# zengyan-97/X2-VLM

Measured on AMD Instinct MI355X. Metric: image-text pairs/sec (fwd+bwd) X2VLM-base 224px bs=64/GPU, higher is better.
Workload: dtype bf16

## Files before the change

include/x2vlm_hip.h:

```cpp
#ifndef X2VLM_HIP_H
#define X2VLM_HIP_H
#include <stdint.h>
#ifdef __cplusplus
extern "C" {
#endif

const char* x2_last_error(void);
int x2_abi_version(void);
int x2_device_cus(void);
int x2_tune(int key, int value);
int x2_tune_get(int key);

int x2_gemm_nt(const void* A, const void* B, void* C, int M, int N, int K, int lda, int ldb, int ldc,
               const float* bias, const float* gamma, const float* resid, int ldr, void* aux, int ldaux,
               int act, int out_f32, unsigned drop_thr16, unsigned drop_seed, float drop_scale, const unsigned* drop_epoch,
               const float* rowscale, float* colsum, void* stream);

int x2_gemm_nt_dgelu_colparts(const void* A, const void* B, void* C, int M, int N, int K, int lda, int ldb, int ldc,
                              const void* aux, int ldaux, float* colparts, int* nrows_out, void* stream);
int x2_gemm_nt_splitk(const void* A, const void* B, float* C, int M, int N, int K, int lda, int ldb, int ldc,
                      int slices, float* ws, long ws_floats, void* stream);

int x2_gemm_tn_grouped(const int64_t* problems, int count, int accumulate, int split, float* ws, long ws_floats,
                       void* stream);
// ... 27 lines not shown

int x2_layernorm_fwd(const float* x, const float* w, const float* b, void* y_bf16, float* y_f32, float* mean,
                     float* rstd, int rows, int D, float eps, int period, unsigned drop_thr16, unsigned drop_seed,
                     float drop_scale, const unsigned* drop_epoch, void* stream);
int x2_layernorm_bwd(const void* dy , int dy_is_bf16, const float* x, const float* mean, const float* rstd, const float* w,
                     const float* dres, float* dx, void* dx_bf16, float* dw, float* db, float* dcol, int rows, int D,
                     int period, unsigned in_thr16, unsigned in_seed, float in_scale, unsigned out_thr16,
                     unsigned out_seed, float out_scale, const unsigned* drop_epoch, float* ws ,
                     int defer, int post, const float* post_rowscale, void* stream);
int x2_colsum_bf16(const void* y, float* out, int M, int N, int ld, float* ws , int defer, void* stream);
int x2_reduce_partials(const float* part, int nblk, int nk, int width, float* o0, float* o1, float* o2, void* stream);
int x2_reduce_partials_multi(const int64_t* desc, int count, void* stream);
int x2_layerscale_finish(const int64_t* desc, int count, void* stream);
int x2_rowscale_cast_colsum(const float* dx, const float* rowscale, void* dx_bf16, float* colsum, int M, int D,
                            float* ws , int defer, void* stream);
int x2_cast_bf16(const float* src, void* dst, long n, void* stream);
int x2_cast_transpose_bf16(const float* src, void* dst, void* dstT, int R, int C, int ldt, void* stream);
int x2_cast_transpose_multi(const int64_t* desc, int count, void* stream);
int x2_copy_f32_multi(const int64_t* desc, int count, void* stream);
int x2_patchify(const float* image, void* cols, int B, int R, int ps, void* stream);
int x2_assemble_tokens(const float* patch, const float* cls, float* x, int B, int P, int D, void* stream);
int x2_assemble_tokens_bwd(const float* dx, void* dpatch_bf16, float* dcls, int B, int P, int D, void* stream);
int x2_pool_tokens(float* x, const float* w, int B, int P, int D, int bwd, void* stream);
int x2_relpos_bias(const float* table, const long* index, const long* indexT , float* bias, float* biasT, int N, int H, int ld, int ldT,
                   float scale, void* stream);
int x2_relpos_bias_bwd(const void* dS, const int* inv_off, const int* inv_pos, float* dtable, int B, int N, int H, int ld,
                       int T, float* ws, int slices, void* stream);

int x2_embed_fwd(const long* ids, const float* word, const float* pos, const float* type0, float* out, int R, int L,
                 int D, void* stream);
int x2_embed_bwd(const long* ids, const float* g, float* dword, float* dpos, float* dtype0, int R, int L, int D,
                 float* scratch, void* stream);
int x2_gather_rows(const float* src, const int* idx, float* dst, void* dst_bf16, int R, long len, void* stream);
int x2_scatter_rows(const float* src, const int* idx, float* dst, int R, int D, long len, void* stream);
int x2_linear_f32(const float* A, const float* B, float* C, const float* bias, const float* alpha_ptr, float alpha,
                  int M, int N, int K, long sam, long sak, long sbn, long sbk, long ldc, int accumulate,
                  int ksplit ,
                  float* ws , void* stream);
int x2_l2norm(const float* x, const float* dy, float* out, int R, int D, int bwd, void* stream);
int x2_ce_fwd(const float* logits, long ld, const long* labels, int R, int C, float* lse, float* loss_row, float* out2,
              void* stream);
int x2_ce_bwd(const float* logits, long ld, const long* labels, const float* lse, const float* g, const float* stat,
              float gscale, int R, int C, float* dl_f32, void* dl_bf16, long ldd, void* stream);
int x2_mlm_ce_fwd(const void* X, const void* E, const float* bias, const long* labels, int R, int Vp, int V, int Hd,
                  int ldx, int lde, float* part, float* zlab, void* stream);
int x2_ce_combine(const float* part, int chunks, const float* zlab, const long* labels, int R, float* lse, float* loss_row,
                  float* out2, void* stream);
int x2_mlm_ce_bwd(const void* X, const void* E, const float* bias, const long* labels, const float* lse, const float* g,
                  const float* stat, float gscale, int R, int Vp, int V, int Hd, int ldx, int lde, void* dl_bf16, long ldd,
                  void* stream);
int x2_mask_tokens(const long* text_ids, const long* text_atts, int B, int L, const unsigned char* is_subword, int vocab,
                   const unsigned* words, int words_ld, unsigned seed, const unsigned* epoch, double mask_prob, int max_masks,
                   double skipgram_prb, int skipgram_size, int mask_whole_word, long cls_id, long mask_id, long pad_id, long pad_mask,
                   long* text_ids_masked, long* masked_pos, long* masked_ids, void* stream);
int x2_sample_negatives(const float* sim, int n, const long* group, const float* u, int* out, void* stream);
int x2_additive_mask(const long* atts, float* out, int S, int L, int Lp, float neg, void* stream);

// ... 40 lines not shown
```

probes/aten_count.py:

```python
import collections
import sqlite3
import sys

db = sqlite3.connect(sys.argv[1])
rows = list(db.execute("select name, start, end from kernels order by start"))
starts = [i for i, r in enumerate(rows) if r[0].startswith("patchify_kernel")]
a, b = starts[-2], starts[-1]
ours, aten = collections.Counter(), collections.Counter()
t_ours = t_aten = 0.0
for n, s, e in rows[a:b]:
    short = n.split("(")[0].replace("void ", "")
    if short.startswith("at::") or "rocclr" in short or short.startswith("Cijk") or "elementwise" in short:
        aten[short[:100]] += 1; t_aten += (e - s) / 1e3
    else:
        ours[short.split("<")[0]] += 1; t_ours += (e - s) / 1e3
print("# one step (the last complete one): %d launches, %d hand-written HIP (%.2f ms), %d ATen / runtime (%.3f ms)"
      % (b - a, sum(ours.values()), t_ours / 1e3, sum(aten.values()), t_aten / 1e3))
for n, k in aten.most_common():
    print("%4d  %s" % (k, n))
```

x2-vlm_amd/_lib.py:

```python
import ctypes as C
import os

import torch

_HERE = os.path.dirname(os.path.abspath(__file__))
LIB_PATH = os.environ.get("X2VLM_HIP_LIB") or os.path.join(_HERE, "libx2vlm_hip.so")

P, I, L, F, U = C.c_void_p, C.c_int, C.c_long, C.c_float, C.c_uint


class AttnArgs(C.Structure):
    _fields_ = [(n, P) for n in ("Q", "K", "V", "O", "dO", "Out", "dQ", "dK", "dV", "dS", "LSE", "Delta")] + \
               [(n, L) for n in ("q_bs", "q_rs", "k_bs", "k_rs", "v_bs", "v_rs", "o_bs", "o_rs",
                                 "dq_bs", "dq_rs", "dk_bs", "dk_rs", "dv_bs", "dv_rs", "do_bs", "do_rs")] + \
               [(n, I) for n in ("B", "Bkv", "H", "Lq", "Lk")] + [("scale", F)] + \
               [("bias", P), ("bias_ld", I), ("biasT", P), ("biasT_ld", I), ("mask", P), ("mask_ld", I),
                ("kv_idx", P), ("seq_off", P), ("seq_ids", P), ("ds_ld", I),
                ("drop_thr16", C.c_uint), ("drop_seed", C.c_uint), ("drop_scale", F), ("dbg", I), ("head_dim", I), ("drop_epoch", P),
                ("grid_nx", I), ("grid_ny", I), ("grid_nz", I), ("grid_map", I),
                ("phase", I), ("ws", P), ("ws_floats", L), ("colsum_ws", P)]


_SIGS = {
    "x2_gemm_nt": [P, P, P, I, I, I, I, I, I, P, P, P, I, P, I, I, I, U, U, F, P, P, P, P],
# ... 29 lines not shown
    "x2_ce_bwd": [P, L, P, P, P, P, F, I, I, P, P, L, P],
    "x2_mlm_ce_fwd": [P, P, P, P, I, I, I, I, I, I, P, P, P],
    "x2_ce_combine": [P, I, P, P, I, P, P, P, P],
    "x2_mlm_ce_bwd": [P, P, P, P, P, P, P, F, I, I, I, I, I, I, P, L, P],
    "x2_sample_negatives": [P, I, P, P, P, P],
    "x2_mask_tokens": [P, P, I, I, P, I, P, I, U, P, C.c_double, I, C.c_double, I, I, L, L, L, L, P, P, P, P],
    "x2_additive_mask": [P, P, I, I, I, F, P],
    "x2_kv_csr": [P, I, I, P, P, P],
    "x2_tail_index": [P, P, P, P, I, I, I, I, P, P, P, P, P],
    "x2_droppath_rows": [P, U, P, I, I, I, P, P],
    "x2_frame_mean": [P, P, P, P, P, I, I, I, I, I, P],
    "x2_gelu_f32": [P, P, P, L, P],
    "x2_grad_norm": [P, I, I, F, P, P, P],
    "x2_adamw_multi": [P, I, I, P, P, I, F, F, F, P, P],
    "x2_colsum_f32": [P, P, I, I, P],
    "x2_attn_fwd_mask2d": [C.POINTER(AttnArgs), P, I, P],
    "x2_attn_bwd_mask2d": [C.POINTER(AttnArgs), P, I, P],
    "x2_additive_mask2d": [P, P, I, I, I, F, P],
    "x2_embed_fwd_pid": [P, P, P, P, P, P, I, I, P],
    "x2_embed_bwd_pid": [P, P, P, P, P, P, I, I, I, P, P],
    "x2_mlm_ls_fwd": [P, P, P, P, L, I, I, I, I, I, I, P, P, P, P, P],
    "x2_ls_combine": [P, P, I, P, P, P, P, I, I, L, F, P, P, P, P],
    "x2_mlm_ls_bwd": [P, P, P, P, P, P, P, P, F, F, L, I, I, I, I, I, I, P, L, P],
}
_COMM_SIGS = {
    "x2_comm_unique_id": [P],
    "x2_comm_init": [P, I, I, C.POINTER(P)],
    "x2_comm_info": [P, C.POINTER(I), C.POINTER(I)],
    "x2_comm_allreduce_bucket": [P, P, L, I, I, P, P],
    "x2_comm_allgather": [P, P, P, L, I, P, P],
    "x2_comm_broadcast": [P, P, L, I, I, P, P],
    "x2_comm_destroy": [P],
}
EXPORTS = sorted(list(_SIGS) + list(_COMM_SIGS) + ["x2_last_error", "x2_abi_version", "x2_device_cus", "x2_tune", "x2_tune_get",
                                                         "x2_attn_bwd_one_pass"])

_lib = None


class X2HipError(RuntimeError):
    pass


def lib():
    global _lib
    if _lib is None:
# ... 42 lines not shown
```

x2-vlm_amd/csrc/heads.hip:

```cpp
#include "x2_common.h"
#define SCATTER_MAX_R_E 8192

__global__ __launch_bounds__(256) void embed_fwd_kernel(const long* __restrict__ ids, const float* __restrict__ word,
                                                        const float* __restrict__ pos, const float* __restrict__ type0,
                                                        float* __restrict__ out, int R, int L, int D) {
  const int r = blockIdx.x;
  const long id = ids[r];
  const int l = r % L;
  for (int d = threadIdx.x * 4; d < D; d += 1024) {
    const float4 a = *reinterpret_cast<const float4*>(word + id * D + d), b = *reinterpret_cast<const float4*>(pos + (long)l * D + d),
                 c = *reinterpret_cast<const float4*>(type0 + d);
    *reinterpret_cast<float4*>(out + (long)r * D + d) = float4{a.x + b.x + c.x, a.y + b.y + c.y, a.z + b.z + c.z, a.w + b.w + c.w};
  }
}
extern "C" int x2_embed_fwd(const long* ids, const float* word, const float* pos, const float* type0, float* out, int R, int L, int D,
                            void* stream) {
  X2_REQUIRE(R > 0 && L > 0 && D % 4 == 0, "x2_embed_fwd: R=%d L=%d D=%d", R, L, D);
  hipLaunchKernelGGL(embed_fwd_kernel, dim3(R), dim3(256), 0, (hipStream_t)stream, ids, word, pos, type0, out, R, L, D);
  return x2_check_launch("x2_embed_fwd");
}
__global__ __launch_bounds__(1024) void embed_bwd_word_kernel(const long* __restrict__ ids, const float* __restrict__ g, float* dword, int R,
                                                              int D) {
  __shared__ uint32_t bm[SCATTER_MAX_R_E / 32];
  __shared__ uint16_t lst[SCATTER_MAX_R_E];
// ... 79 lines not shown
  float* p = dpos + (long)l * D + d;
  p[0] += t.x; p[1] += t.y; p[2] += t.z; p[3] += t.w;
  *reinterpret_cast<float4*>(tot + (long)l * D + d) = t;
}
__global__ __launch_bounds__(64) void embed_bwd_type_kernel(const float* __restrict__ tot, float* dtype0, int L, int D) {
  const int d = (blockIdx.x * 64 + threadIdx.x) * 4;
  if (d >= D) return;
  float4 t{0.f, 0.f, 0.f, 0.f};
  for (int l = 0; l < L; ++l) { const float4 v = *reinterpret_cast<const float4*>(tot + (long)l * D + d); t.x += v.x; t.y += v.y; t.z += v.z; t.w += v.w; }
  float4 o = *reinterpret_cast<float4*>(dtype0 + d);
  o.x += t.x; o.y += t.y; o.z += t.z; o.w += t.w;
  *reinterpret_cast<float4*>(dtype0 + d) = o;
}
extern "C" int x2_embed_bwd(const long* ids, const float* g, float* dword, float* dpos, float* dtype0, int R, int L, int D, float* scratch,
                            void* stream) {
  X2_REQUIRE(R > 0 && L > 0 && D % 4 == 0 && D <= 4096 && scratch, "x2_embed_bwd: R=%d L=%d D=%d (D <= 4096, scratch of min(L, R) * D floats)", R, L, D);
  hipLaunchKernelGGL(embed_bwd_word_kernel, dim3(R), dim3(1024), 0, (hipStream_t)stream, ids, g, dword, R, D);
  const int Lp = L < R ? L : R;
  hipLaunchKernelGGL(embed_bwd_pos_kernel, dim3(Lp, (D / 4 + 255) / 256), dim3(256), 0, (hipStream_t)stream, g, dpos, scratch, R, L, D);
  hipLaunchKernelGGL(embed_bwd_type_kernel, dim3((D / 4 + 63) / 64), dim3(64), 0, (hipStream_t)stream, scratch, dtype0, Lp, D);
  return x2_check_launch("x2_embed_bwd");
}

__global__ __launch_bounds__(256) void gather_rows_kernel(const float* __restrict__ src, const int* __restrict__ idx, float* dst,
                                                          bf16_t* dstb, long len) {
  const long r = blockIdx.y;
  const float* s = src + (long)idx[r] * len;
  for (long e = (blockIdx.x * 256L + threadIdx.x) * 4; e < len; e += (long)gridDim.x * 1024) {
    const float4 v = *reinterpret_cast<const float4*>(s + e);
    if (dst) *reinterpret_cast<float4*>(dst + r * len + e) = v;
    if (dstb) *reinterpret_cast<u32x2*>(dstb + r * len + e) = u32x2{pack_bf16(v.x, v.y), pack_bf16(v.z, v.w)};
  }
}
extern "C" int x2_gather_rows(const float* src, const int* idx, float* dst, void* dst_bf16, int R, long len, void* stream) {
  X2_REQUIRE(R > 0 && len > 0 && len % 4 == 0, "x2_gather_rows: R=%d len=%ld", R, len);
  const int bx = (int)((len / 4 + 255) / 256 < 64 ? (len / 4 + 255) / 256 : 64);
  hipLaunchKernelGGL(gather_rows_kernel, dim3(bx, R), dim3(256), 0, (hipStream_t)stream, src, idx, dst, (bf16_t*)dst_bf16, len);
  return x2_check_launch("x2_gather_rows");
}
#define SCATTER_MAX_R 8192
__global__ __launch_bounds__(256) void scatter_rows_kernel(const float* __restrict__ src, const int* __restrict__ idx, float* __restrict__ dst,
                                                           int R, long len, int chunks) {
  __shared__ uint32_t bm[SCATTER_MAX_R / 32];
  const int d = blockIdx.x / chunks;
  const long e = ((long)(blockIdx.x % chunks) * 256L + threadIdx.x) * 4;
  float4 acc{0.f, 0.f, 0.f, 0.f};
// ... 501 lines not shown
```

x2-vlm_amd/csrc/rowwise.hip:

```cpp
#include "x2_common.h"

__device__ __forceinline__ long remap_row(int r, int period) { return period > 0 ? (long)r + r / period + 1 : r; }

#define LN_MAXV 8
#define LN_DISPATCH(D, CALL) do { const int nv_ = ((D) + 255) / 256; \
  if (nv_ <= 1) { CALL(1); } else if (nv_ == 2) { CALL(2); } else if (nv_ == 3) { CALL(3); } else if (nv_ == 4) { CALL(4); } \
  else if (nv_ <= 6) { CALL(6); } else { CALL(8); } } while (0)
template <int NV>
__global__ __launch_bounds__(256) void layernorm_fwd_kernel(const float* __restrict__ x, const float* __restrict__ w,
                                                            const float* __restrict__ bsh, bf16_t* yb, float* yf,
                                                            float* mean, float* rstd, int rows, int D, float eps, int period,
                                                            DropSpec drop_in_, const uint32_t* __restrict__ epoch) {
  const int row = blockIdx.x * 4 + (threadIdx.x >> 6), lane = threadIdx.x & 63;
  if (row >= rows) return;
  const DropSpec drop = drop_at_epoch(drop_in_, epoch);
  const long gr = remap_row(row, period);
  const float* xr = x + gr * D;
  float4 v[NV];
  float s = 0.f;
  const int nv = D >> 2;
#pragma unroll
  for (int i = 0; i < NV; ++i) {
    const int c = lane + i * 64;
    if (c < nv) { v[i] = *reinterpret_cast<const float4*>(xr + c * 4); s += v[i].x + v[i].y + v[i].z + v[i].w; }
// ... 648 lines not shown
}
__global__ __launch_bounds__(64) void cls_grad_kernel(const float* __restrict__ dx, float* dcls, int B, long bstride, int D) {
  const int d = (blockIdx.x * 64 + threadIdx.x) * 4;
  if (d >= D) return;
  float4 t{0.f, 0.f, 0.f, 0.f};
#pragma unroll 8
  for (int b = 0; b < B; ++b) {
    const float4 v = *reinterpret_cast<const float4*>(dx + b * bstride + d);
    t.x += v.x; t.y += v.y; t.z += v.z; t.w += v.w;
  }
  float4 o = *reinterpret_cast<float4*>(dcls + d);
  o.x += t.x; o.y += t.y; o.z += t.z; o.w += t.w;
  *reinterpret_cast<float4*>(dcls + d) = o;
}
extern "C" int x2_assemble_tokens_bwd(const float* dx, void* dpatch, float* dcls, int B, int P, int D, void* stream) {
  X2_REQUIRE(B > 0 && P > 0 && D % 4 == 0, "x2_assemble_tokens_bwd: B=%d P=%d D=%d", B, P, D);
  const long total = (long)B * (P + 1) * D / 4;
  const int blocks = (int)((total + 255) / 256 < 8192 ? (total + 255) / 256 : 8192);
  hipLaunchKernelGGL(assemble_tokens_bwd_kernel, dim3(blocks), dim3(256), 0, (hipStream_t)stream, dx, (bf16_t*)dpatch, dcls, B, P, D);
  hipLaunchKernelGGL(cls_grad_kernel, dim3((D / 4 + 63) / 64), dim3(64), 0, (hipStream_t)stream, dx, dcls, B, (long)(P + 1) * D, D);
  return x2_check_launch("x2_assemble_tokens_bwd");
}

__global__ __launch_bounds__(256) void pool_tokens_kernel(float* x, const float* __restrict__ w, int B, int P, int D, int bwd) {
  __shared__ float4 part[3][64];
  __shared__ float wpart[4];
  const int b = blockIdx.x, lane = threadIdx.x & 63, wave = threadIdx.x >> 6;
  const int d = (blockIdx.y * 64 + lane) * 4;
  const bool live = d < D;
  float* xb = x + (long)b * (P + 1) * D;
  float wsum = (float)P;
  if (w) {
    float s = 0.f;
    for (int p = threadIdx.x; p < P; p += 256) s += w[(long)b * P + p];
    s = wave_sum(s);
    if (lane == 0) wpart[wave] = s;
    __syncthreads();
    wsum = wpart[0] + wpart[1] + wpart[2] + wpart[3];
  }
  const float inv = 1.f / wsum;
  if (!bwd) {
    float4 acc{0.f, 0.f, 0.f, 0.f};
    if (live)
      for (int p = wave; p < P; p += 4) {
        const float wp = w ? w[(long)b * P + p] : 1.f;
        const float4 v = *reinterpret_cast<const float4*>(xb + (long)(1 + p) * D + d);
        acc.x += wp * v.x; acc.y += wp * v.y; acc.z += wp * v.z; acc.w += wp * v.w;
      }
    if (wave > 0) part[wave - 1][lane] = acc;
    __syncthreads();
    if (wave == 0 && live) {
#pragma unroll
      for (int k = 0; k < 3; ++k) { const float4 o = part[k][lane]; acc.x += o.x; acc.y += o.y; acc.z += o.z; acc.w += o.w; }
      *reinterpret_cast<float4*>(xb + d) = float4{acc.x * inv, acc.y * inv, acc.z * inv, acc.w * inv};
    }
  } else {
    if (live) {
      const float4 g0 = *reinterpret_cast<const float4*>(xb + d);
      for (int p = wave; p < P; p += 4) {
        const float wp = (w ? w[(long)b * P + p] : 1.f) * inv;
        float4 v = *reinterpret_cast<float4*>(xb + (long)(1 + p) * D + d);
        v.x += wp * g0.x; v.y += wp * g0.y; v.z += wp * g0.z; v.w += wp * g0.w;
        *reinterpret_cast<float4*>(xb + (long)(1 + p) * D + d) = v;
      }
    }
    __syncthreads();
    if (wave == 0 && live) *reinterpret_cast<float4*>(xb + d) = float4{0.f, 0.f, 0.f, 0.f};
  }
}
extern "C" int x2_pool_tokens(float* x, const float* w, int B, int P, int D, int bwd, void* stream) {
  X2_REQUIRE(B > 0 && P > 0 && D % 4 == 0, "x2_pool_tokens: B=%d P=%d D=%d", B, P, D);
  hipLaunchKernelGGL(pool_tokens_kernel, dim3(B, (D + 255) / 256), dim3(256), 0, (hipStream_t)stream, x, w, B, P, D, bwd);
  return x2_check_launch("x2_pool_tokens");
}

__global__ __launch_bounds__(256) void relpos_bias_kernel(const float* __restrict__ table, const long* __restrict__ index,
                                                          const long* __restrict__ indexT, float* bias, float* biasT, int N, int H,
                                                          int ld, int ldT, float scale) {
  const long total = (long)N * N;
  long e = blockIdx.x * 256L + threadIdx.x;
  if (e >= total) return;
  const int i = (int)(e / N), j = (int)(e % N);
  const long idx = index[e];
  if (indexT && biasT) {
    const long idt = indexT[e];
    for (int h = 0; h < H; ++h) {
      bias[((long)h * N + i) * ld + j] = table[idx * H + h] * scale;
      biasT[((long)h * N + i) * ldT + j] = table[idt * H + h] * scale;
    }
    return;
  }
  for (int h = 0; h < H; ++h) {
    const float v = table[idx * H + h] * scale;
    bias[((long)h * N + i) * ld + j] = v;
    if (biasT) biasT[((long)h * N + j) * ldT + i] = v;
  }
// ... 59 lines not shown
```

x2-vlm_amd/engine.py:

```python
import itertools
import math
import os
import weakref

import torch

from . import kernels as K
from ._lib import raw_stream

BF16, F32 = torch.bfloat16, torch.float32



_SERIAL = itertools.count(1)


def _tok(w):
    t = w.__dict__.get("_x2_serial")
    if t is None:
        t = w.__dict__["_x2_serial"] = next(_SERIAL)
    return t


class TScale:
# ... 434 lines not shown
            _count_call(("vit", id(p["blocks.%d.gamma_1" % i])))
        if stem:
            _count_call(("vit-stem", id(p["cls_token"])))
        ctx.meta, ctx.saved, ctx.final, ctx.cols = meta, saved, final, cols
        ctx.params = params
        ctx.dims = (B, P_, T, H, D, M, scale)
        return out

    @staticmethod
    def backward(ctx, dout):
        meta, params = ctx.meta, ctx.params
        BANK.note_backward()
        depth = meta["depth"]
        lo, hi = meta.get("lo", 0), meta.get("hi", depth)
        stem, head = lo == 0, hi == depth
        names = vision_param_names(depth, lo, hi)
        p = dict(zip(names, params))
        B, P_, T, H, D, M, scale = ctx.dims
        dev = dout.device
        out = {}
        if head:
            x_last, meanf, rstdf = ctx.final
            hn = ("fc_norm.weight", "fc_norm.bias")
            Gh = Grads(dev, [(n, p[n].shape, True) for n in hn], key=("vit-head", id(p["fc_norm.weight"])), params=[p[n] for n in hn])
            g = dout.contiguous().clone()
            K.pool_tokens(g, meta.get("pool_w"), bwd=True)
            dx, _ = K.layernorm_bwd(g.view(M, D), x_last, meanf, rstdf, p["fc_norm.weight"], Gh["fc_norm.weight"], Gh["fc_norm.bias"],
                                    period=P_)
            Gh.publish()
            out.update(Gh.g)
        else:
            dx = dout.contiguous().view(M, D)
        dS = torch.empty(B, H, T, K.round_up(T, 64), device=dev, dtype=BF16) if hi > lo else None
        F4 = p["blocks.%d.mlp.fc1.weight" % lo].shape[0] if hi > lo else 0
        dpath = meta.get("drop_path")
        pairs = _LayerPairs()
        arenas = {}
        for i in range(lo, hi):
            b = "blocks.%d." % i
            arenas[i] = Grads(dev, [("gamma_1", (D,), True), ("gamma_2", (D,), True), ("norm1.weight", (D,), True), ("norm1.bias", (D,), True),
                                    ("qkv_bias", (3 * D,), True), ("attn.relative_position_bias_table", p[b + "attn.relative_position_bias_table"].shape, True),
                                    ("attn.proj.bias", (D,), True), ("norm2.weight", (D,), True), ("norm2.bias", (D,), True),
                                    ("mlp.fc1.bias", (F4,), True), ("mlp.fc2.bias", (D,), True),
                                    ("_cs1", (D,), True), ("_cs2", (D,), True),
                                    ("attn.qkv.weight", (3 * D, D), False), ("attn.proj.weight", (D, D), False),
                                    ("mlp.fc1.weight", (F4, D), False), ("mlp.fc2.weight", (D, F4), False)], key=("vit", id(p[b + "gamma_1"])),
                              params=[p[n] for n in names if n.startswith(b)], zero=False)
        Gs = None
        if stem:
            sn = ("cls_token", "patch_embed.proj.weight", "patch_embed.proj.bias")
            Gs = Grads(dev, [(n, p[n].shape, True) for n in sn], key=("vit-stem", id(p["cls_token"])), params=[p[n] for n in sn], zero=False)
        Grads.zero_all(list(arenas.values()) + ([Gs] if Gs is not None else []))
        dxb = None
        for i in reversed(range(lo, hi)):
            b = "blocks.%d." % i
            rs1, rs2 = dpath[i] if dpath is not None else (None, None)
            (x, h1, mean1, rstd1, qkv, bias, biasT, att, lse, x1, h2, mean2, rstd2, pre, act) = ctx.saved[i - lo]
            ctx.saved[i - lo] = None
            G = arenas.pop(i)
            _begin_layer_backward()
            _, w2T = BANK.linear(p[b + "mlp.fc2.weight"], tscale=p[b + "gamma_2"])
            _, w1T = BANK.linear(p[b + "mlp.fc1.weight"])
            _, wprojT = BANK.linear(p[b + "attn.proj.weight"], tscale=p[b + "gamma_1"])
            _, wqkvT = BANK.linear(p[b + "attn.qkv.weight"])
            if dxb is None:
                dxb = K.rowscale_cast_colsum(dx, G["_cs2"], rowscale=rs2)
            if FUSE_DGELU_COLSUM:
                dpre = K.gemm_nt_dgelu_colsum(dxb, w2T, pre, G["mlp.fc1.bias"])
            else:
                dpre = K.gemm_nt(dxb, w2T, aux=pre, act=2)
                K.colsum_bf16(dpre, G["mlp.fc1.bias"])
            dh2 = K.gemm_nt(dpre, w1T)
            dx1, dx1b = K.layernorm_bwd(dh2, x1, mean2, rstd2, p[b + "norm2.weight"], G["norm2.weight"], G["norm2.bias"], dres=dx,
                                        post=(rs1, G["_cs1"]))
            datt = K.gemm_nt(dx1b, wprojT)
# ... 317 lines not shown



class EmbeddingsFn(torch.autograd.Function):

    @staticmethod
    def forward(ctx, ids, eps, drop, word, pos, typ, lnw, lnb, pids=None):
        S, L = ids.shape
        ids = ids.contiguous()
        if pids is not None:
            pids = pids.to(torch.int64).expand(S, L).contiguous()
            e = K.embed_fwd_pid(ids, pids, word.detach(), pos.detach(), typ.detach())
        else:
            e = K.embed_fwd(ids, word.detach(), pos.detach(), typ.detach())
        _, y, mean, rstd = K.layernorm_fwd(e, lnw, lnb, eps, want_bf16=False, want_f32=True, drop=drop)
        ctx.save_for_backward(ids, e, mean, rstd, word, pos, typ, lnw)
        ctx.drop, ctx.pids = drop, pids
        return y.view(S, L, -1)

    @staticmethod
    def backward(ctx, dy):
        ids, e, mean, rstd, word, pos, typ, lnw = ctx.saved_tensors
        n = lnw.numel()
        zeros = torch.zeros(2 * n + pos.numel() + typ.numel(), device=dy.device, dtype=F32)
        dw, db = zeros[:n], zeros[n:2 * n]
        dpos, dtyp = zeros[2 * n:2 * n + pos.numel()].view_as(pos), zeros[2 * n + pos.numel():].view_as(typ)
        de, _ = K.layernorm_bwd(dy.contiguous().view(e.shape), e, mean, rstd, lnw, dw, db, drop_in=ctx.drop)
        dword = _TIED_DWORD.pop(_tok(word), None)
        if dword is None:
            dword = torch.zeros_like(word)
        if ctx.pids is not None:
            K.embed_bwd_pid(ids, ctx.pids, de, dword, dpos, dtyp)
        else:
            K.embed_bwd(ids, de, dword, dpos, dtyp)
        return None, None, None, dword, dpos, dtyp, dw, db, None



class MlmLossFn(torch.autograd.Function):

    @staticmethod
    def forward(ctx, rows, labels, eps, keep_logits, dw_, db_, lnw, lnb, dec_bias, word, smooth=None):
        R, Hd = rows.shape
        V = word.shape[0]
        rb = K.cast_bf16(rows.contiguous())
        wd, _ = BANK.linear(dw_)
        t_pre = torch.empty(R, Hd, device=rows.device, dtype=BF16)
# ... 162 lines not shown
    @staticmethod
    def backward(ctx, g):
        logits, labels, lse, stat = ctx.saved_tensors
        return K.ce_bwd(logits, labels, lse, g.reshape(1).to(F32).contiguous(), stat), None


class GatherRowsFn(torch.autograd.Function):

    @staticmethod
    def forward(ctx, src, idx):
        src = src.contiguous()
        row_len = src[0].numel()
        ctx.save_for_backward(idx)
        ctx.shape = src.shape
        out, _ = K.gather_rows(src.view(src.shape[0], row_len), idx, row_len)
        return out.view((idx.numel(),) + src.shape[1:])

    @staticmethod
    def backward(ctx, dy):
        (idx,) = ctx.saved_tensors
        row_len = dy[0].numel()
        dst = K.scatter_rows(dy.contiguous().view(idx.numel(), row_len), idx, ctx.shape[0], row_len)
        return dst.view(ctx.shape), None
```

x2-vlm_amd/graph.py:

```python
import gc
import os

import torch

from . import kernels as K


class GraphedStep:
    def __init__(self, fn, warmup=2, enabled=True, verbose=False):
        self.fn, self.graph, self.out = fn, None, None
        self._grads = []
        self.stream = torch.cuda.Stream()
        self.mode = "eager"
        self.error = None
        self._epoch = None
        if not enabled or os.environ.get("X2_GRAPH", "1") == "0":
            return
        from . import engine
        if K.DROP_EPOCH is None:
            K.DROP_EPOCH = torch.zeros(1, dtype=torch.int32, device="cuda")
        self._epoch = K.DROP_EPOCH
        side_rule, engine.SIDE.only_from = engine.SIDE.only_from, self.stream.cuda_stream
        try:
            gc.collect()
# ... 271 lines not shown
        if hasattr(te, "cls"):
            eng.BANK.linear(te.cls.predictions.transform.dense.weight)
            eng.BANK.vocab(bert.embeddings.word_embeddings.weight)

    def _s_vision(self):
        b = self.batch
        enc = self.model.vision_encoder
        self.t["vmid"] = []
        enc.chunk_at, enc.chunk_hook = self.vcuts, self._vhook
        try:
            self.t["vis"] = self.model.tower_vision(b["image"], b.get("image_atts"), b.get("idx_to_group_img"), self.ret_bbox_loss)
        finally:
            enc.chunk_at, enc.chunk_hook = None, None

    def _s_feat(self):
        m = self.model
        if self.clamp_temp and isinstance(m.temp, torch.nn.Parameter):
            with torch.no_grad():
                m.temp.clamp_(0.001, 0.5)
        ie, _, full = self.t["vis"]
        self.t["ie"] = ie.detach().requires_grad_()
        self.t["full"] = None if full is None else full.detach().requires_grad_()
        self.t["both_leaf"] = self.t["both"].detach().requires_grad_()
        self.t["feat"] = m.tail_features(self.t["ie"], self.t["both_leaf"])

    def _gather(self):
        fi, ft = self.t["feat"]
        if not self.coll:
            for src, dst in ((fi, self.t["fi_all"]), (ft, self.t["ft_all"])):
                dst.detach().copy_(src.detach())
            return
        self.sG.wait_stream(self.sA)
        with torch.cuda.stream(self.sG):
            for src, dst in ((fi, self.t["fi_all"]), (ft, self.t["ft_all"])):
                out = dst.detach()
                if self.comm is not None:
                    self.comm.allgather(src.detach().contiguous(), out)
                else:
                    import torch.distributed as dist
                    dist.all_gather(list(out.chunk(self.world)), src.detach().contiguous(), group=self.pg)
                self.messages += 1
        self.sA.wait_stream(self.sG)

    def _s_loss(self):
        m, b, t = self.model, self.batch, self.t
        for leaf in (t["fi_all"], t["ft_all"], t["ie"], t["both_leaf"], t["full"]):
            if leaf is not None:
                leaf.grad = None
        fi, ft = t["feat"]
        loss = m.tail_losses(t["ie"], t["vis"][1], t["both_leaf"], fi, ft, b["text_atts"], b["masked_pos"], b["masked_ids"],
                             image_embeds_fullatts=t["full"], target_bbox=b.get("target_bbox"), is_image=b.get("is_image"),
                             ret_bbox_loss=self.ret_bbox_loss, ret_match_loss=self.ret_match_loss,
                             gathered=(t["fi_all"], t["ft_all"]))
        self._backward(loss)
        B = fi.shape[0]
        sl = slice(self.rank * B, (self.rank + 1) * B)
        if t["fi_all"].grad is not None:
            torch.autograd.backward([fi, ft], [t["fi_all"].grad[sl], t["ft_all"].grad[sl]])
        t["loss"] = {k: v.detach() for k, v in loss.items()}

    def _backward(self, losses):
        tot = self.total_loss(losses)
        if torch.is_tensor(tot) and tot.requires_grad:
            tot.backward()

    def _s_vision_bwd(self, ci=0):
        if ci == 0:
            ie_out, _, full_out = self.t["vis"]
            pairs = [(ie_out, self.t["ie"].grad)]
            if full_out is not None:
                pairs.append((full_out, self.t["full"].grad))
        else:
            x, leaf = self.t["vmid"][len(self.vcuts) - ci]
            pairs = [(x, leaf.grad)]
        pairs = [(o, g) for o, g in pairs if g is not None]
        if pairs:
            torch.autograd.backward([o for o, _ in pairs], [g for _, g in pairs])

    def _s_vision_wgrad(self, ci):
        work = self._vq.pop(ci, None)
        self._held.append(work)
# ... 399 lines not shown
```

x2-vlm_amd/kernels.py:

```python
import ctypes as C

import torch

from . import _lib
from ._lib import AttnArgs, call, ptr, raw_stream

BF16, F32 = torch.bfloat16, torch.float32


GEMM_TIMER = None


class _timed:

    def __init__(self, flops, name="gemm_nt"):
        self.flops = flops
        self.name = name

    def __enter__(self):
        if GEMM_TIMER is not None:
            self.a = torch.cuda.Event(enable_timing=True)
            self.b = torch.cuda.Event(enable_timing=True)
            self.a.record()

# ... 377 lines not shown


def assemble_tokens(patch, cls, B, P):
    D = patch.shape[1]
    x = torch.empty(B, P + 1, D, device=patch.device, dtype=F32)
    call("x2_assemble_tokens", ptr(patch), ptr(cls), ptr(x), B, P, D)
    return x


def assemble_tokens_bwd(dx, dcls):
    B, T, D = dx.shape
    dpatch = torch.empty(B * (T - 1), D, device=dx.device, dtype=BF16)
    call("x2_assemble_tokens_bwd", ptr(dx), ptr(dpatch), ptr(dcls), B, T - 1, D)
    return dpatch


def pool_tokens(x, w=None, bwd=False):
    B, T, D = x.shape
    assert x.dtype == F32 and x.is_contiguous() and (w is None or (w.dtype == F32 and w.shape == (B, T - 1) and w.is_contiguous()))
    call("x2_pool_tokens", ptr(x), ptr(w), B, T - 1, D, 1 if bwd else 0)
    return x


LOG2E = 1.4426950408889634


def relpos_bias(table, index, want_T=True, log2=False):
    N = index.shape[0]
    H = table.shape[1]
    ld = round_up(N, 64)
    bias = torch.empty(H, N, ld, device=table.device, dtype=F32)
    biasT = torch.empty(H, N, ld, device=table.device, dtype=F32) if want_T else None
    call("x2_relpos_bias", ptr(table), ptr(index), ptr(_relpos_index_t(index)) if want_T else None, ptr(bias), ptr(biasT), N, H, ld, ld,
         LOG2E if log2 else 1.0)
    return bias, biasT


_RELPOS_CSR = {}
_RELPOS_T = {}


def _relpos_index_t(index):
    key = (index.data_ptr(), index._version)
    ent = _RELPOS_T.get(key)
    if ent is None:
        ent = _RELPOS_T[key] = (index.t().contiguous(), index)
# ... 301 lines not shown
```

x2-vlm_amd/model_pretrain.py:

```python
import torch

from . import kernels as K
from . import ops
from .xvlm import XVLMBase


class XVLM(XVLMBase):
    def __init__(self, config, load_vision_params=True, load_text_params=True, pretraining=True):
        super().__init__(config, load_vision_params=load_vision_params, load_text_params=load_text_params,
                         use_contrastive_loss=True, use_matching_loss=True, use_mlm_loss=True, use_bbox_loss=True,
                         config_text=None, pretraining=pretraining)
        self.overlap_towers = True
        self._text_stream = None

    def tower_text(self, text_ids, text_atts, text_ids_masked):
        return self.get_text_embeds(torch.cat([text_ids, text_ids_masked]), torch.cat([text_atts, text_atts]))

    def tower_vision(self, image, image_atts=None, idx_to_group_img=None, ret_bbox_loss=False):
        if ret_bbox_loss:
            return self.get_vision_embeds(image, image_atts=image_atts, idx_to_group_img=idx_to_group_img)
        return self.get_vision_embeds(image) + (None,)

    def tail_features(self, image_embeds, both):
        return self.get_features(image_embeds, both[:image_embeds.shape[0]])

    def tail_losses(self, image_embeds, image_atts, both, image_feat, text_feat, text_atts, masked_pos, masked_ids,
                    image_embeds_fullatts=None, target_bbox=None, is_image=None, ret_bbox_loss=False, ret_match_loss=True,
                    gathered=None):
        B = image_embeds.shape[0]
        dev = both.device
        text_embeds = both[:B]
        loss_itc = self.get_contrastive_loss(image_feat, text_feat, gathered=gathered)
        ineg, tneg = self.get_hard_negatives(image_feat, text_feat) if ret_match_loss else (None, None)
        if both.is_cuda:
            t_idx, kv, atts, enc_atts = K.tail_index(ineg, tneg, text_atts.contiguous(), image_atts.contiguous(), with_match=ret_match_loss)
        else:
            ar = torch.arange(B, device=dev, dtype=torch.int32)
            t_idx, kv = (torch.cat([ar, ar, tneg, ar + B]), torch.cat([ar, ineg, ar, ar])) if ret_match_loss else (ar + B, ar)
            atts, enc_atts = torch.cat([text_atts, text_atts])[t_idx.long()], image_atts[kv.long()]
        h0 = ops.gather_rows(both, t_idx)
        fused = self.get_cross_embeds(image_embeds, enc_atts, text_embeds=h0, text_atts=atts, kv_idx=kv)
        if ret_match_loss:
            loss_itm = self._itm_loss(fused[:3 * B, 0, :], B)
        else:
            loss_itm = torch.tensor(0.0)
        loss_mlm, self.last_mlm_lse, self.last_mlm_logits = self.text_encoder.mlm_loss_from_hidden(fused[-B:], masked_pos, masked_ids)
        loss = {"loss_itc": loss_itc, "loss_itm": loss_itm, "loss_mlm": loss_mlm}
        self.last = dict(image_embeds=image_embeds.detach(), text_embeds=text_embeds.detach(), image_feat=image_feat.detach(),
                         text_feat=text_feat.detach())
        if ret_bbox_loss:
            output_coord = self.predict_bbox(image_embeds_fullatts, text_embeds, text_atts)
            self.last["bbox_coord"] = output_coord.detach()
            loss["loss_bbox"], loss["loss_giou"] = self.get_bbox_loss(output_coord, target_bbox, is_image=is_image)
        return loss

    def forward_multimodal(self, image, text_ids, text_atts, text_ids_masked=None, masked_pos=None, masked_ids=None,
                           image_atts=None, idx_to_group_img=None, target_bbox=None, is_image=None,
                           ret_bbox_loss=False, ret_match_loss=True):
        overlap = self.overlap_towers and image.is_cuda
        if overlap:
            if self._text_stream is None:
                self._text_stream = torch.cuda.Stream()
            main = torch.cuda.current_stream()
            self._text_stream.wait_stream(main)
            with torch.cuda.stream(self._text_stream):
                both = self.tower_text(text_ids, text_atts, text_ids_masked)
        image_embeds, image_atts, image_embeds_fullatts = self.tower_vision(image, image_atts, idx_to_group_img, ret_bbox_loss)
        if overlap:
            main.wait_stream(self._text_stream)
# ... 22 lines not shown
```

Baseline: 2970.

## Replace ATen slicing/clone/zero ops around heads with custom fused HIP kernels

Adds custom kernels to remove leftover ATen launches: pool-token backward now writes to a separate buffer and zeroes the dx row in the same pass, which replaces the clone. Slicing the fused output into CLS rows and the MLM tail now goes through a custom autograd function, so backward is one kernel instead of ATen scatter and zero-fill. The ITC features take CLS leaves, with a token-0 add into the tower grads. Embedding grad zeroing now goes through the batched zero_all, and probes are added to list the ATen call sites. This cuts the number of small launches per step, at the cost of more custom paths that must keep gradients exact.

```diff
diff --git a/include/x2vlm_hip.h b/include/x2vlm_hip.h
--- a/include/x2vlm_hip.h
+++ b/include/x2vlm_hip.h
@@ -73,6 +73,7 @@
 int x2_assemble_tokens(const float* patch, const float* cls, float* x, int B, int P, int D, void* stream);
 int x2_assemble_tokens_bwd(const float* dx, void* dpatch_bf16, float* dcls, int B, int P, int D, void* stream);
 int x2_pool_tokens(float* x, const float* w, int B, int P, int D, int bwd, void* stream);
+int x2_pool_tokens_bwd_to(const float* g, float* out, float* zero0, const float* w, int B, int P, int D, void* stream);
 int x2_relpos_bias(const float* table, const long* index, const long* indexT , float* bias, float* biasT, int N, int H, int ld, int ldT,
                    float scale, void* stream);
 int x2_relpos_bias_bwd(const void* dS, const int* inv_off, const int* inv_pos, float* dtable, int B, int N, int H, int ld,
@@ -84,6 +85,8 @@
                  float* scratch, void* stream);
 int x2_gather_rows(const float* src, const int* idx, float* dst, void* dst_bf16, int R, long len, void* stream);
 int x2_scatter_rows(const float* src, const int* idx, float* dst, int R, int D, long len, void* stream);
+int x2_split_tokens_bwd(const float* dcls, const float* dtail, float* out, int S, int n_cls, int L, int D, void* stream);
+int x2_add_token0(float* x, const float* rows, int B, int T, int D, void* stream);
 int x2_linear_f32(const float* A, const float* B, float* C, const float* bias, const float* alpha_ptr, float alpha,
                   int M, int N, int K, long sam, long sak, long sbn, long sbk, long ldc, int accumulate,
                   int ksplit ,
diff --git a/probes/aten_count.py b/probes/aten_count.py
--- a/probes/aten_count.py
+++ b/probes/aten_count.py
@@ -3,18 +3,25 @@
 import sys
 
 db = sqlite3.connect(sys.argv[1])
-rows = list(db.execute("select name, start, end from kernels order by start"))
+rows = list(db.execute("select name, start, end, stream_id from kernels order by start"))
 starts = [i for i, r in enumerate(rows) if r[0].startswith("patchify_kernel")]
 a, b = starts[-2], starts[-1]
 ours, aten = collections.Counter(), collections.Counter()
 t_ours = t_aten = 0.0
-for n, s, e in rows[a:b]:
+listing, prev = [], "-"
+for n, s, e, sid in rows[a:b]:
     short = n.split("(")[0].replace("void ", "")
     if short.startswith("at::") or "rocclr" in short or short.startswith("Cijk") or "elementwise" in short:
         aten[short[:100]] += 1; t_aten += (e - s) / 1e3
+        listing.append("%8.3f ms %6.1f us  stream %s  %-72s after %s" % ((s - rows[a][1]) / 1e6, (e - s) / 1e3, sid,
+                                                                          short.replace("at::native::", "")[:72], prev))
     else:
         ours[short.split("<")[0]] += 1; t_ours += (e - s) / 1e3
+        prev = short.split("<")[0]
 print("# one step (the last complete one): %d launches, %d hand-written HIP (%.2f ms), %d ATen / runtime (%.3f ms)"
       % (b - a, sum(ours.values()), t_ours / 1e3, sum(aten.values()), t_aten / 1e3))
 for n, k in aten.most_common():
     print("%4d  %s" % (k, n))
+if "--list" in sys.argv[2:]:
+    print("# offset, duration, stream, kernel, preceding hand-written kernel")
+    print("\n".join(listing))
diff --git a/probes/aten_sites.py b/probes/aten_sites.py
--- /dev/null
+++ b/probes/aten_sites.py
@@ -0,0 +1,82 @@
+import argparse
+import collections
+import importlib
+import os
+import sys
+import tempfile
+import traceback
+
+import torch
+from torch.utils._python_dispatch import TorchDispatchMode
+
+ROOT = os.path.dirname(os.path.dirname(os.path.abspath(__file__)))
+sys.path.insert(0, ROOT)
+import bench
+
+NO_KERNEL = ("empty", "new_empty", "empty_like", "empty_strided", "detach", "alias", "record_stream", "_local_scalar_dense", "lift_fresh",
+             "is_pinned", "_to_copy.host")
+
+
+def main():
+    ap = argparse.ArgumentParser()
+    ap.add_argument("--config", default="base")
+    args = ap.parse_args()
+    conf = bench.CONFIGS[args.config]
+    dev = torch.device("cuda", 0)
+    mp = importlib.import_module("x2-vlm_amd.model_pretrain")
+    cfgs = importlib.import_module("x2-vlm_amd.configs")
+    graph = importlib.import_module("x2-vlm_amd.graph")
+    synth = importlib.import_module("x2-vlm_amd.synthetic")
+    torch.manual_seed(0)
+    cfg = cfgs.pretrain_config(tempfile.mkdtemp(), conf["size"], conf["res"])
+    model = mp.XVLM(config=cfg, load_vision_params=False, load_text_params=False, pretraining=True).to(dev)
+    model.train()
+    batch = {k: v.to(dev) for k, v in bench.synthetic_batch(0, conf["batch"], 30, conf["res"], frames=conf["frames"]).items()}
+    masking = synth.masking_config({}, synth.synth_subword_flags(30522).to(dev), seed=1234)
+    runner = graph.SegmentedStep(model, batch, warmup=2, enabled=False, masking=masking)
+
+    seg = ["-"]
+    inner = runner._seg
+
+    def _seg(mode, name, stream, fn, pool):
+        seg[0] = name
+        try:
+            inner(mode, name, stream, fn, pool)
+        finally:
+            seg[0] = "between"
+    runner._seg = _seg
+    rec = collections.OrderedDict()
+
+    class Rec(TorchDispatchMode):
+        def __torch_dispatch__(self, func, types, args=(), kwargs=None):
+            out = func(*args, **(kwargs or {}))
+            name = str(func).replace("aten.", "")
+            if any(r.alias_info is not None and not r.alias_info.is_write for r in func._schema.returns) or name.split(".")[0] in NO_KERNEL:
+                return out
+            outs = out if isinstance(out, (tuple, list)) else (out,)
+            ts = [t for t in outs if torch.is_tensor(t)]
+            if not any(t.is_cuda for t in ts) and not any(torch.is_tensor(a) and a.is_cuda for a in args):
+                return out
+            site = "(autograd engine)"
+            for fr in reversed(traceback.extract_stack()):
+                if "x2-vlm_amd" in fr.filename:
+                    site = "%s:%d" % (os.path.basename(fr.filename), fr.lineno)
+                    break
+            nbytes = sum(t.numel() * t.element_size() for t in ts)
+            key = (seg[0], name, site, nbytes, " ".join("x".join(map(str, t.shape)) or "scalar" for t in ts))
+            rec[key] = rec.get(key, 0) + 1
+            return out
+
+    with Rec():
+        runner()
+    torch.cuda.synchronize()
+    print("# segment | op | site | output bytes | output shape | calls")
+    tot = collections.Counter()
+    for (s, name, site, nbytes, shape), n in rec.items():
+        print("%-8s %-28s %-24s %10d  %-18s x%d" % (s, name, site, nbytes, shape, n))
+        tot[s] += n
+    print("# ops per segment: " + ", ".join("%s %d" % kv for kv in tot.items()))
+
+
+if __name__ == "__main__":
+    main()
diff --git a/x2-vlm_amd/_lib.py b/x2-vlm_amd/_lib.py
--- a/x2-vlm_amd/_lib.py
+++ b/x2-vlm_amd/_lib.py
@@ -75,6 +75,9 @@
     "x2_mlm_ls_fwd": [P, P, P, P, L, I, I, I, I, I, I, P, P, P, P, P],
     "x2_ls_combine": [P, P, I, P, P, P, P, I, I, L, F, P, P, P, P],
     "x2_mlm_ls_bwd": [P, P, P, P, P, P, P, P, F, F, L, I, I, I, I, I, I, P, L, P],
+    "x2_pool_tokens_bwd_to": [P, P, P, P, I, I, I, P],
+    "x2_split_tokens_bwd": [P, P, P, I, I, I, I, P],
+    "x2_add_token0": [P, P, I, I, I, P],
 }
 _COMM_SIGS = {
     "x2_comm_unique_id": [P],
diff --git a/x2-vlm_amd/csrc/heads.hip b/x2-vlm_amd/csrc/heads.hip
--- a/x2-vlm_amd/csrc/heads.hip
+++ b/x2-vlm_amd/csrc/heads.hip
@@ -125,6 +125,45 @@
   return x2_check_launch("x2_embed_bwd");
 }
 
+__global__ __launch_bounds__(256) void split_tokens_bwd_kernel(const float* __restrict__ dcls, const float* __restrict__ dtail, float* __restrict__ out,
+                                                               int S, int n_cls, int L, int D) {
+  const long total = (long)S * L * D / 4;
+  const long st = (long)gridDim.x * 256;
+  for (long i = blockIdx.x * 256L + threadIdx.x; i < total; i += st) {
+    const long e = i * 4;
+    const int d = (int)(e % D);
+    const long row = e / D;
+    const int l = (int)(row % L), s = (int)(row / L);
+    float4 v{0.f, 0.f, 0.f, 0.f};
+    if (s >= n_cls) { if (dtail) v = *reinterpret_cast<const float4*>(dtail + e - (long)n_cls * L * D); }
+    else if (l == 0 && dcls) v = *reinterpret_cast<const float4*>(dcls + (long)s * D + d);
+    *reinterpret_cast<float4*>(out + e) = float4{v.x + 0.f, v.y + 0.f, v.z + 0.f, v.w + 0.f};
+  }
+}
+extern "C" int x2_split_tokens_bwd(const float* dcls, const float* dtail, float* out, int S, int n_cls, int L, int D, void* stream) {
+  X2_REQUIRE(out && S > 0 && L > 0 && D > 0 && D % 4 == 0 && n_cls >= 0 && n_cls <= S, "x2_split_tokens_bwd: S=%d n_cls=%d L=%d D=%d", S, n_cls, L, D);
+  const long total = (long)S * L * D / 4;
+  const int blocks = (int)((total + 255) / 256 < 8192 ? (total + 255) / 256 : 8192);
+  hipLaunchKernelGGL(split_tokens_bwd_kernel, dim3(blocks), dim3(256), 0, (hipStream_t)stream, dcls, dtail, out, S, n_cls, L, D);
+  return x2_check_launch("x2_split_tokens_bwd");
+}
+
+__global__ __launch_bounds__(256) void add_token0_kernel(float* x, const float* __restrict__ rows, int B, long bstride, int D) {
+  const long i = (blockIdx.x * 256L + threadIdx.x) * 4;
+  if (i >= (long)B * D) return;
+  const int b = (int)(i / D), d = (int)(i % D);
+  float4 a = *reinterpret_cast<float4*>(x + b * bstride + d);
+  const float4 r = *reinterpret_cast<const float4*>(rows + i);
+  a.x += r.x; a.y += r.y; a.z += r.z; a.w += r.w;
+  *reinterpret_cast<float4*>(x + b * bstride + d) = a;
+}
+extern "C" int x2_add_token0(float* x, const float* rows, int B, int T, int D, void* stream) {
+  X2_REQUIRE(x && rows && B > 0 && T > 0 && D > 0 && D % 4 == 0, "x2_add_token0: x=%p rows=%p B=%d T=%d D=%d", (void*)x, (const void*)rows, B, T, D);
+  const long n4 = (long)B * D / 4;
+  hipLaunchKernelGGL(add_token0_kernel, dim3((unsigned)((n4 + 255) / 256)), dim3(256), 0, (hipStream_t)stream, x, rows, B, (long)T * D, D);
+  return x2_check_launch("x2_add_token0");
+}
+
 __global__ __launch_bounds__(256) void gather_rows_kernel(const float* __restrict__ src, const int* __restrict__ idx, float* dst,
                                                           bf16_t* dstb, long len) {
   const long r = blockIdx.y;
diff --git a/x2-vlm_amd/csrc/rowwise.hip b/x2-vlm_amd/csrc/rowwise.hip
--- a/x2-vlm_amd/csrc/rowwise.hip
+++ b/x2-vlm_amd/csrc/rowwise.hip
@@ -694,13 +694,15 @@
   return x2_check_launch("x2_assemble_tokens_bwd");
 }
 
-__global__ __launch_bounds__(256) void pool_tokens_kernel(float* x, const float* __restrict__ w, int B, int P, int D, int bwd) {
+__global__ __launch_bounds__(256) void pool_tokens_kernel(const float* src, float* x, float* zero0, const float* __restrict__ w, int B, int P,
+                                                          int D, int bwd) {
   __shared__ float4 part[3][64];
   __shared__ float wpart[4];
   const int b = blockIdx.x, lane = threadIdx.x & 63, wave = threadIdx.x >> 6;
   const int d = (blockIdx.y * 64 + lane) * 4;
   const bool live = d < D;
   float* xb = x + (long)b * (P + 1) * D;
+  const float* sb = src + (long)b * (P + 1) * D;
   float wsum = (float)P;
   if (w) {
     float s = 0.f;
@@ -728,22 +730,30 @@
     }
   } else {
     if (live) {
-      const float4 g0 = *reinterpret_cast<const float4*>(xb + d);
+      const float4 g0 = *reinterpret_cast<const float4*>(sb + d);
       for (int p = wave; p < P; p += 4) {
         const float wp = (w ? w[(long)b * P + p] : 1.f) * inv;
-        float4 v = *reinterpret_cast<float4*>(xb + (long)(1 + p) * D + d);
+        float4 v = *reinterpret_cast<const float4*>(sb + (long)(1 + p) * D + d);
         v.x += wp * g0.x; v.y += wp * g0.y; v.z += wp * g0.z; v.w += wp * g0.w;
         *reinterpret_cast<float4*>(xb + (long)(1 + p) * D + d) = v;
       }
     }
     __syncthreads();
-    if (wave == 0 && live) *reinterpret_cast<float4*>(xb + d) = float4{0.f, 0.f, 0.f, 0.f};
+    if (wave == 0 && live) {
+      *reinterpret_cast<float4*>(xb + d) = float4{0.f, 0.f, 0.f, 0.f};
+      if (zero0) *reinterpret_cast<float4*>(zero0 + (long)b * (P + 1) * D + d) = float4{0.f, 0.f, 0.f, 0.f};
+    }
   }
 }
 extern "C" int x2_pool_tokens(float* x, const float* w, int B, int P, int D, int bwd, void* stream) {
-  X2_REQUIRE(B > 0 && P > 0 && D % 4 == 0, "x2_pool_tokens: B=%d P=%d D=%d", B, P, D);
-  hipLaunchKernelGGL(pool_tokens_kernel, dim3(B, (D + 255) / 256), dim3(256), 0, (hipStream_t)stream, x, w, B, P, D, bwd);
+  X2_REQUIRE(x && B > 0 && P > 0 && D % 4 == 0, "x2_pool_tokens: B=%d P=%d D=%d", B, P, D);
+  hipLaunchKernelGGL(pool_tokens_kernel, dim3(B, (D + 255) / 256), dim3(256), 0, (hipStream_t)stream, (const float*)x, x, (float*)nullptr, w, B, P, D, bwd);
   return x2_check_launch("x2_pool_tokens");
+}
+extern "C" int x2_pool_tokens_bwd_to(const float* g, float* out, float* zero0, const float* w, int B, int P, int D, void* stream) {
+  X2_REQUIRE(g && out && B > 0 && P > 0 && D % 4 == 0, "x2_pool_tokens_bwd_to: g=%p out=%p B=%d P=%d D=%d", (const void*)g, (void*)out, B, P, D);
+  hipLaunchKernelGGL(pool_tokens_kernel, dim3(B, (D + 255) / 256), dim3(256), 0, (hipStream_t)stream, g, out, zero0, w, B, P, D, 1);
+  return x2_check_launch("x2_pool_tokens_bwd_to");
 }
 
 __global__ __launch_bounds__(256) void relpos_bias_kernel(const float* __restrict__ table, const long* __restrict__ index,
diff --git a/x2-vlm_amd/engine.py b/x2-vlm_amd/engine.py
--- a/x2-vlm_amd/engine.py
+++ b/x2-vlm_amd/engine.py
@@ -480,15 +480,7 @@
         if head:
             x_last, meanf, rstdf = ctx.final
             hn = ("fc_norm.weight", "fc_norm.bias")
-            Gh = Grads(dev, [(n, p[n].shape, True) for n in hn], key=("vit-head", id(p["fc_norm.weight"])), params=[p[n] for n in hn])
-            g = dout.contiguous().clone()
-            K.pool_tokens(g, meta.get("pool_w"), bwd=True)
-            dx, _ = K.layernorm_bwd(g.view(M, D), x_last, meanf, rstdf, p["fc_norm.weight"], Gh["fc_norm.weight"], Gh["fc_norm.bias"],
-                                    period=P_)
-            Gh.publish()
-            out.update(Gh.g)
-        else:
-            dx = dout.contiguous().view(M, D)
+            Gh = Grads(dev, [(n, p[n].shape, True) for n in hn], key=("vit-head", id(p["fc_norm.weight"])), params=[p[n] for n in hn], zero=False)
         dS = torch.empty(B, H, T, K.round_up(T, 64), device=dev, dtype=BF16) if hi > lo else None
         F4 = p["blocks.%d.mlp.fc1.weight" % lo].shape[0] if hi > lo else 0
         dpath = meta.get("drop_path")
@@ -508,7 +500,15 @@
         if stem:
             sn = ("cls_token", "patch_embed.proj.weight", "patch_embed.proj.bias")
             Gs = Grads(dev, [(n, p[n].shape, True) for n in sn], key=("vit-stem", id(p["cls_token"])), params=[p[n] for n in sn], zero=False)
-        Grads.zero_all(list(arenas.values()) + ([Gs] if Gs is not None else []))
+        Grads.zero_all(([Gh] if head else []) + list(arenas.values()) + ([Gs] if Gs is not None else []))
+        if head:
+            dx = torch.empty(M, D, device=dev, dtype=F32)
+            g = K.pool_tokens_bwd_to(dout.contiguous(), meta.get("pool_w"), zero0=dx)
+            K.layernorm_bwd(g.view(M, D), x_last, meanf, rstdf, p["fc_norm.weight"], Gh["fc_norm.weight"], Gh["fc_norm.bias"], period=P_, dx=dx)
+            Gh.publish()
+            out.update(Gh.g)
+        else:
+            dx = dout.contiguous().view(M, D)
         dxb = None
         for i in reversed(range(lo, hi)):
             b = "blocks.%d." % i
@@ -872,7 +872,8 @@
     def backward(ctx, dy):
         ids, e, mean, rstd, word, pos, typ, lnw = ctx.saved_tensors
         n = lnw.numel()
-        zeros = torch.zeros(2 * n + pos.numel() + typ.numel(), device=dy.device, dtype=F32)
+        zeros = torch.empty(2 * n + pos.numel() + typ.numel(), device=dy.device, dtype=F32)
+        Grads.zero_all([], extra=[zeros])
         dw, db = zeros[:n], zeros[n:2 * n]
         dpos, dtyp = zeros[2 * n:2 * n + pos.numel()].view_as(pos), zeros[2 * n + pos.numel():].view_as(typ)
         de, _ = K.layernorm_bwd(dy.contiguous().view(e.shape), e, mean, rstd, lnw, dw, db, drop_in=ctx.drop)
@@ -1081,3 +1082,27 @@
         row_len = dy[0].numel()
         dst = K.scatter_rows(dy.contiguous().view(idx.numel(), row_len), idx, ctx.shape[0], row_len)
         return dst.view(ctx.shape), None
+
+
+class SplitFusedFn(torch.autograd.Function):
+
+    _IDX = {}
+
+    @staticmethod
+    def forward(ctx, fused, n_cls):
+        S, L, D = fused.shape
+        fused = fused.contiguous()
+        key = (n_cls, L, fused.device)
+        idx = SplitFusedFn._IDX.get(key)
+        if idx is None:
+            idx = SplitFusedFn._IDX[key] = (torch.arange(n_cls, dtype=torch.int32) * L).to(fused.device)
+        ctx.dims = (S, n_cls, L, D)
+        cls = K.gather_rows(fused.view(S * L, D), idx, D)[0] if n_cls else fused.new_empty(0, D)
+        return cls, fused[n_cls:]
+
+    @staticmethod
+    def backward(ctx, dcls, dtail):
+        S, n_cls, L, D = ctx.dims
+        dev = (dcls if dcls is not None else dtail).device
+        return K.split_tokens_bwd(None if dcls is None else dcls.contiguous(), None if dtail is None else dtail.contiguous(),
+                                  S, n_cls, L, D, dev), None
diff --git a/x2-vlm_amd/graph.py b/x2-vlm_amd/graph.py
--- a/x2-vlm_amd/graph.py
+++ b/x2-vlm_amd/graph.py
@@ -317,7 +317,11 @@
         self.t["ie"] = ie.detach().requires_grad_()
         self.t["full"] = None if full is None else full.detach().requires_grad_()
         self.t["both_leaf"] = self.t["both"].detach().requires_grad_()
-        self.t["feat"] = m.tail_features(self.t["ie"], self.t["both_leaf"])
+        B = ie.shape[0]
+        self.t["cls_leaf"] = None
+        if ie.is_cuda and ie.dim() == 3:
+            self.t["cls_leaf"] = (ie.detach()[:, 0, :].requires_grad_(), self.t["both"].detach()[:B, 0, :].requires_grad_())
+        self.t["feat"] = m.tail_features(self.t["ie"], self.t["both_leaf"], cls=self.t["cls_leaf"])
 
     def _gather(self):
         fi, ft = self.t["feat"]
@@ -339,7 +343,7 @@
 
     def _s_loss(self):
         m, b, t = self.model, self.batch, self.t
-        for leaf in (t["fi_all"], t["ft_all"], t["ie"], t["both_leaf"], t["full"]):
+        for leaf in (t["fi_all"], t["ft_all"], t["ie"], t["both_leaf"], t["full"]) + tuple(t["cls_leaf"] or ()):
             if leaf is not None:
                 leaf.grad = None
         fi, ft = t["feat"]
@@ -352,6 +356,11 @@
         sl = slice(self.rank * B, (self.rank + 1) * B)
         if t["fi_all"].grad is not None:
             torch.autograd.backward([fi, ft], [t["fi_all"].grad[sl], t["ft_all"].grad[sl]])
+            for leaf, tower in zip(t["cls_leaf"] or (), (t["ie"], t["both_leaf"])):
+                if leaf.grad is not None:
+                    if tower.grad is None:
+                        tower.grad = torch.zeros_like(tower)
+                    K.add_token0(tower.grad, leaf.grad.contiguous())
         t["loss"] = {k: v.detach() for k, v in loss.items()}
 
     def _backward(self, losses):
diff --git a/x2-vlm_amd/kernels.py b/x2-vlm_amd/kernels.py
--- a/x2-vlm_amd/kernels.py
+++ b/x2-vlm_amd/kernels.py
@@ -423,6 +423,31 @@
     return x
 
 
+def pool_tokens_bwd_to(g, w=None, zero0=None):
+    B, T, D = g.shape
+    assert g.dtype == F32 and g.is_contiguous() and (w is None or (w.dtype == F32 and w.shape == (B, T - 1) and w.is_contiguous()))
+    assert zero0 is None or (zero0.dtype == F32 and zero0.is_contiguous() and zero0.numel() == g.numel())
+    out = torch.empty_like(g)
+    call("x2_pool_tokens_bwd_to", ptr(g), ptr(out), ptr(zero0), ptr(w), B, T - 1, D)
+    return out
+
+
+def split_tokens_bwd(dcls, dtail, S, n_cls, L, D, device):
+    for t, shape in ((dcls, (n_cls, D)), (dtail, (S - n_cls, L, D))):
+        assert t is None or (t.dtype == F32 and t.is_contiguous() and tuple(t.shape) == shape), (None if t is None else t.shape, shape)
+    out = torch.empty(S, L, D, device=device, dtype=F32)
+    call("x2_split_tokens_bwd", ptr(dcls), ptr(dtail), ptr(out), S, n_cls, L, D)
+    return out
+
+
+def add_token0(x, rows):
+    B, D = rows.shape
+    assert x.dtype == F32 and rows.dtype == F32 and x.is_contiguous() and rows.is_contiguous() and x.dim() == 3
+    assert x.shape[0] >= B and x.shape[2] == D and D % 4 == 0
+    call("x2_add_token0", ptr(x), ptr(rows), B, x.shape[1], D)
+    return x
+
+
 LOG2E = 1.4426950408889634
 
 
diff --git a/x2-vlm_amd/model_pretrain.py b/x2-vlm_amd/model_pretrain.py
--- a/x2-vlm_amd/model_pretrain.py
+++ b/x2-vlm_amd/model_pretrain.py
@@ -2,6 +2,7 @@
 
 from . import kernels as K
 from . import ops
+from .engine import SplitFusedFn
 from .xvlm import XVLMBase
 
 
@@ -21,7 +22,9 @@
             return self.get_vision_embeds(image, image_atts=image_atts, idx_to_group_img=idx_to_group_img)
         return self.get_vision_embeds(image) + (None,)
 
-    def tail_features(self, image_embeds, both):
+    def tail_features(self, image_embeds, both, cls=None):
+        if cls is not None:
+            return tuple(ops.normalize(ops.linear(x, proj.weight, proj.bias)) for x, proj in zip(cls, (self.vision_proj, self.text_proj)))
         return self.get_features(image_embeds, both[:image_embeds.shape[0]])
 
     def tail_losses(self, image_embeds, image_atts, both, image_feat, text_feat, text_atts, masked_pos, masked_ids,
@@ -41,10 +44,11 @@
         h0 = ops.gather_rows(both, t_idx)
         fused = self.get_cross_embeds(image_embeds, enc_atts, text_embeds=h0, text_atts=atts, kv_idx=kv)
         if ret_match_loss:
-            loss_itm = self._itm_loss(fused[:3 * B, 0, :], B)
+            cls, masked = SplitFusedFn.apply(fused, 3 * B) if fused.is_cuda else (fused[:3 * B, 0, :], fused[-B:])
+            loss_itm = self._itm_loss(cls, B)
         else:
-            loss_itm = torch.tensor(0.0)
-        loss_mlm, self.last_mlm_lse, self.last_mlm_logits = self.text_encoder.mlm_loss_from_hidden(fused[-B:], masked_pos, masked_ids)
+            loss_itm, masked = torch.tensor(0.0), fused[-B:]
+        loss_mlm, self.last_mlm_lse, self.last_mlm_logits = self.text_encoder.mlm_loss_from_hidden(masked, masked_pos, masked_ids)
         loss = {"loss_itc": loss_itc, "loss_itm": loss_itm, "loss_mlm": loss_mlm}
         self.last = dict(image_embeds=image_embeds.detach(), text_embeds=text_embeds.detach(), image_feat=image_feat.detach(),
                          text_feat=text_feat.detach())
```

Result: no change. 2981, median of 4 (+0.4%).
